# heliaxdev/ark-plonk

Hardware: AMD Instinct MI355X
Metric: proofs/sec at 2^20 constraints (BLS12-381, KZG10); MSM G1-adds/s (higher is better)
Workload: dtype u32 limbs (256/384-bit Montgomery integers)

## Files before the change

ark_plonk_amd/csrc/ecu.cuh:

```cuda
#pragma once
#include "fields.cuh"

template <class F>
struct AffineU {
    F x, y;
    ZK_HD bool is_null() const { return x.limbs_zero() && y.limbs_zero(); }
};

template <class F>
struct XYZZu {
    F x, y, zz, zzz;

    ZK_HD static XYZZu infinity() {
        XYZZu r;
        r.x = F::zero();
        r.y = F::zero();
        r.zz = F::zero();
        r.zzz = F::zero();
        return r;
    }
    ZK_HD bool is_inf() const { return zz.limbs_zero(); }

    ZK_HD static XYZZu from_affine(const AffineU<F>& p) {
        XYZZu r;
        r.x = p.x;
        r.y = p.y;
        r.zz = F::one();
        r.zzz = F::one();
        return r;
    }

    ZK_HD static XYZZu dbl_affine(const AffineU<F>& p) {
        F u = F::dbl(p.y);
        F v = F::sqr(u);
        F w = F::mul(u, v);
        F s = F::mul(p.x, v);
        F xx = F::sqr(p.x);
        F m = F::add3(xx, xx, xx);
        XYZZu r;
        r.x = F::sub8(F::sqr(m), F::dbl(s));
        r.y = F::dot2(m, F::sub16(s, r.x), w, F::neg16(p.y));
        r.zz = v;
        r.zzz = w;
        return r;
    }

    ZK_HD static XYZZu dbl(const XYZZu& p) {
        if (p.is_inf()) return p;
        F u = F::dbl(p.y);
        F v = F::sqr(u);
        F w = F::mul(u, v);
        F s = F::mul(p.x, v);
        F xx = F::sqr(p.x);
        F m = F::add3(xx, xx, xx);
        XYZZu r;
        r.x = F::sub8(F::sqr(m), F::dbl(s));
        r.y = F::dot2(m, F::sub16(s, r.x), w, F::neg16(p.y));
        r.zz = F::mul(v, p.zz);
        r.zzz = F::mul(w, p.zzz);
        return r;
    }

    ZK_HD static XYZZu madd(const XYZZu& p, const AffineU<F>& q) {
        if (p.is_inf()) return from_affine(q);
        F u2 = F::mul(q.x, p.zz);
        F s2 = F::mul(q.y, p.zzz);
        F pp_ = F::sub16(u2, p.x);
        F r_ = F::sub16(s2, p.y);
        F pp = F::sqr(pp_);
        F rr = F::sqr(r_);
        XYZZu o;
        o.zz = F::mul(p.zz, pp);
        if (o.zz.is_zero_mod_reduced()) {
            if (rr.is_zero_mod_reduced()) return dbl_affine(q);
            return infinity();
        }
        F ppp = F::mul(pp_, pp);
        F qq = F::mul(p.x, pp);
        o.x = F::sub_sum3(rr, ppp, qq, qq);
        o.y = F::dot2(r_, F::sub16(qq, o.x), F::neg16(p.y), ppp);
        o.zzz = F::mul(p.zzz, ppp);
        return o;
    }

    ZK_HD static XYZZu add(const XYZZu& p, const XYZZu& q) {
        if (p.is_inf()) return q;
        if (q.is_inf()) return p;
        F u1 = F::mul(p.x, q.zz);
        F u2 = F::mul(q.x, p.zz);
        F s1 = F::mul(p.y, q.zzz);
        F s2 = F::mul(q.y, p.zzz);
        F pp_ = F::sub8(u2, u1);
        F r_ = F::sub8(s2, s1);
        F pp = F::sqr(pp_);
        F rr = F::sqr(r_);
        XYZZu o;
        o.zz = F::mul(F::mul(p.zz, q.zz), pp);
        if (o.zz.is_zero_mod_reduced()) {
            if (rr.is_zero_mod_reduced()) return dbl(p);
            return infinity();
        }
        F ppp = F::mul(pp_, pp);
        F qq = F::mul(u1, pp);
        o.x = F::sub_sum3(rr, ppp, qq, qq);
        o.y = F::dot2(r_, F::sub16(qq, o.x), F::neg16(s1), ppp);
        o.zzz = F::mul(F::mul(p.zzz, q.zzz), ppp);
        return o;
    }

    ZK_HD bool to_affine(AffineU<F>& out) const {
        if (is_inf()) {
            out.x = F::zero();
            out.y = F::zero();
            return false;
        }
        F i3 = F::inverse(zzz);
        F zi = F::mul(zz, i3);
        F zi2 = F::sqr(zi);
        out.x = F::mul(x, zi2);
        out.y = F::mul(y, i3);
        return true;
    }
};
```

ark_plonk_amd/csrc/fields.cuh:

```cuda
#pragma once
#include "zk_common.h"

template <class P>
struct Fs {
    static constexpr int NL = P::NL;
    static constexpr int SAT = P::SAT_WORDS;
    static constexpr uint32_t M = (1u << 30) - 1u;
    static constexpr int32_t H = 1 << 29;
    uint32_t v[NL];

    ZK_HD static int32_t sx(uint32_t x) { return (int32_t)(x << 2) >> 2; }
    ZK_HD static int64_t column_bias() {
        int64_t h = H;
#if defined(__HIP_DEVICE_COMPILE__)
        asm volatile("" : "+s"(h));
#endif
        return h;
    }

    ZK_HD static Fs zero() {
        Fs r;
#pragma unroll
        for (int i = 0; i < NL; ++i) r.v[i] = 0;
        return r;
    }
    ZK_HD static Fs one() {
        Fs r;
#pragma unroll
        for (int i = 0; i < NL; ++i) r.v[i] = (uint32_t)P::ONE(i);
        return r;
    }
    ZK_HD bool limbs_zero() const {
        uint32_t o = 0;
#pragma unroll
        for (int i = 0; i < NL; ++i) o |= v[i];
        return o == 0;
    }

    ZK_HD static void normalize(Fs& t) {
        int32_t c = 0;
#pragma unroll
        for (int i = 0; i < NL - 1; ++i) {
            const int32_t x = (int32_t)t.v[i];
            const int32_t r = sx((uint32_t)x);
            t.v[i] = (uint32_t)(r + c);
            c = (x - r) >> 30;
        }
        t.v[NL - 1] += (uint32_t)c;
    }
    ZK_HD static void normalize_wide(Fs& t) {
        int32_t c = 0;
#pragma unroll
        for (int i = 0; i < NL - 1; ++i) {
            const int32_t x = (int32_t)t.v[i];
            t.v[i] = (uint32_t)(sx((uint32_t)x) + c);
            c = (x >> 30) + (int32_t)(((uint32_t)x >> 29) & 1u);
        }
        t.v[NL - 1] += (uint32_t)c;
    }
    ZK_HD static void normalize_strict(Fs& t) {
#pragma unroll
        for (int i = 0; i < NL - 1; ++i) {
            const int32_t x = (int32_t)t.v[i];
            const int32_t r = sx((uint32_t)x);
            t.v[i] = (uint32_t)r;
            t.v[i + 1] += (uint32_t)((x - r) >> 30);
        }
    }

    ZK_HD static Fs add(const Fs& a, const Fs& b) {
        Fs t;
#pragma unroll
        for (int i = 0; i < NL; ++i) t.v[i] = a.v[i] + b.v[i];
        normalize(t);
        return t;
    }
    ZK_HD static Fs dbl(const Fs& a) {
        Fs t;
#pragma unroll
        for (int i = 0; i < NL; ++i) t.v[i] = a.v[i] << 1;
        normalize(t);
        return t;
    }
    ZK_HD static Fs add3(const Fs& a, const Fs& b, const Fs& c) {
        Fs t;
#pragma unroll
        for (int i = 0; i < NL; ++i) t.v[i] = a.v[i] + b.v[i] + c.v[i];
        normalize_wide(t);
        return t;
    }
    ZK_HD static Fs sub(const Fs& a, const Fs& b) {
        Fs t;
#pragma unroll
        for (int i = 0; i < NL; ++i) t.v[i] = a.v[i] - b.v[i];
        normalize(t);
        return t;
    }
    ZK_HD static Fs sub_sum3(const Fs& a, const Fs& b, const Fs& c, const Fs& d) {
        Fs t;
#pragma unroll
        for (int i = 0; i < NL; ++i) t.v[i] = a.v[i] - b.v[i] - c.v[i] - d.v[i];
        normalize_wide(t);
        return t;
    }
    ZK_HD static Fs sub2(const Fs& a, const Fs& b) { return sub(a, b); }
    ZK_HD static Fs sub8(const Fs& a, const Fs& b) { return sub(a, b); }
    ZK_HD static Fs sub16(const Fs& a, const Fs& b) { return sub(a, b); }
    ZK_HD static Fs neg16(const Fs& a) {
        Fs t;
#pragma unroll
        for (int i = 0; i < NL; ++i) t.v[i] = 0u - a.v[i];
        return t;
    }
    ZK_HD static Fs neg_canonical(const Fs& a) { return neg16(a); }

    ZK_HD static Fs mul(const Fs& a, const Fs& b) {
        int32_t m[NL];
        Fs r;
        int64_t carry = 0;
        const int64_t hb = column_bias();
#pragma unroll
        for (int k = 0; k < NL; ++k) {
            int64_t a0 = 0, a1 = 0, am = 0;
#pragma unroll
            for (int i = 0; i <= k; ++i) {
                if (i & 1) a1 += (int64_t)(int32_t)a.v[i] * (int32_t)b.v[k - i];
                else a0 += (int64_t)(int32_t)a.v[i] * (int32_t)b.v[k - i];
            }
#pragma unroll
            for (int i = 0; i < k; ++i) am += (int64_t)m[i] * P::MOD(k - i);
            int64_t t = a0 + a1 + am + carry;
            m[k] = (int32_t)((uint32_t)t * (P::PINV << 2)) >> 2;
            t += (int64_t)m[k] * P::MOD(0);
            carry = t >> 30;
        }
#pragma unroll
        for (int k = NL; k < 2 * NL - 1; ++k) {
            int64_t a0 = hb, a1 = 0, am = 0;
#pragma unroll
            for (int i = k - NL + 1; i < NL; ++i) {
                if (i & 1) a1 += (int64_t)(int32_t)a.v[i] * (int32_t)b.v[k - i];
                else a0 += (int64_t)(int32_t)a.v[i] * (int32_t)b.v[k - i];
                am += (int64_t)m[i] * P::MOD(k - i);
            }
            const int64_t t = a0 + a1 + am + carry;
            r.v[k - NL] = ((uint32_t)t & M) - (uint32_t)H;
            carry = t >> 30;
        }
        r.v[NL - 1] = (uint32_t)carry;
        return r;
    }
    ZK_HD static Fs dot2(const Fs& a, const Fs& b, const Fs& c, const Fs& d) {
        int32_t m[NL];
        Fs r;
        int64_t carry = 0;
        const int64_t hb = column_bias();
#pragma unroll
        for (int k = 0; k < NL; ++k) {
            int64_t a0 = 0, a1 = 0, am = 0;
#pragma unroll
            for (int i = 0; i <= k; ++i) {
                a0 += (int64_t)(int32_t)a.v[i] * (int32_t)b.v[k - i];
                a1 += (int64_t)(int32_t)c.v[i] * (int32_t)d.v[k - i];
            }
#pragma unroll
            for (int i = 0; i < k; ++i) am += (int64_t)m[i] * P::MOD(k - i);
            int64_t t = a0 + a1 + am + carry;
            m[k] = (int32_t)((uint32_t)t * (P::PINV << 2)) >> 2;
            t += (int64_t)m[k] * P::MOD(0);
            carry = t >> 30;
        }
#pragma unroll
        for (int k = NL; k < 2 * NL - 1; ++k) {
            int64_t a0 = hb, a1 = 0, am = 0;
#pragma unroll
            for (int i = k - NL + 1; i < NL; ++i) {
                a0 += (int64_t)(int32_t)a.v[i] * (int32_t)b.v[k - i];
                a1 += (int64_t)(int32_t)c.v[i] * (int32_t)d.v[k - i];
                am += (int64_t)m[i] * P::MOD(k - i);
            }
            const int64_t t = a0 + a1 + am + carry;
            r.v[k - NL] = ((uint32_t)t & M) - (uint32_t)H;
            carry = t >> 30;
        }
        r.v[NL - 1] = (uint32_t)carry;
        return r;
    }
    ZK_HD static Fs sqr(const Fs& a) {
        int32_t m[NL], a2[NL];
        Fs r;
#pragma unroll
        for (int i = 0; i < NL; ++i) a2[i] = (int32_t)(a.v[i] << 1);
        int64_t carry = 0;
        const int64_t hb = column_bias();
#pragma unroll
        for (int k = 0; k < NL; ++k) {
            int64_t aa = 0, am = 0;
#pragma unroll
            for (int i = 0; 2 * i < k; ++i) aa += (int64_t)a2[i] * (int32_t)a.v[k - i];
            if ((k & 1) == 0) aa += (int64_t)(int32_t)a.v[k / 2] * (int32_t)a.v[k / 2];
#pragma unroll
            for (int i = 0; i < k; ++i) am += (int64_t)m[i] * P::MOD(k - i);
            int64_t t = aa + am + carry;
            m[k] = (int32_t)((uint32_t)t * (P::PINV << 2)) >> 2;
            t += (int64_t)m[k] * P::MOD(0);
            carry = t >> 30;
        }
#pragma unroll
        for (int k = NL; k < 2 * NL - 1; ++k) {
            int64_t aa = hb, am = 0;
#pragma unroll
            for (int i = k - NL + 1; 2 * i < k; ++i) aa += (int64_t)a2[i] * (int32_t)a.v[k - i];
            if ((k & 1) == 0) aa += (int64_t)(int32_t)a.v[k / 2] * (int32_t)a.v[k / 2];
#pragma unroll
            for (int i = k - NL + 1; i < NL; ++i) am += (int64_t)m[i] * P::MOD(k - i);
            const int64_t t = aa + am + carry;
            r.v[k - NL] = ((uint32_t)t & M) - (uint32_t)H;
            carry = t >> 30;
        }
        r.v[NL - 1] = (uint32_t)carry;
        return r;
    }

    ZK_HD bool is_zero_mod_reduced() const {
        if (v[0] != 0 && v[0] != (uint32_t)P::MOD(0) && v[0] != (uint32_t)P::NMOD(0)) return false;
        uint32_t dz = 0, dp = 0, dn = 0;
#pragma unroll
        for (int i = 0; i < NL; ++i) {
            dz |= v[i];
            dp |= v[i] ^ (uint32_t)P::MOD(i);
            dn |= v[i] ^ (uint32_t)P::NMOD(i);
        }
        return dz == 0 || dp == 0 || dn == 0;
    }
    ZK_HD bool is_zero_mod() const { return mul(*this, one()).is_zero_mod_reduced(); }

    ZK_HD static void floor_sweep(Fs& t) {
#pragma unroll
        for (int i = 0; i < NL - 1; ++i) {
            const int32_t x = (int32_t)t.v[i];
            t.v[i] = (uint32_t)x & M;
            t.v[i + 1] += (uint32_t)(x >> 30);
        }
    }
    ZK_HD static Fs canon_floor(const Fs& a) {
        Fs x = a;
        floor_sweep(x);
#pragma unroll
        for (int it = 0; it < 2; ++it) {
            Fs y;
#pragma unroll
            for (int i = 0; i < NL; ++i) y.v[i] = x.v[i] + (uint32_t)P::MOD(i);
            floor_sweep(y);
            const bool neg = (int32_t)x.v[NL - 1] < 0;
#pragma unroll
            for (int i = 0; i < NL; ++i) x.v[i] = neg ? y.v[i] : x.v[i];
        }
#pragma unroll
        for (int it = 0; it < 2; ++it) {
            Fs y;
#pragma unroll
            for (int i = 0; i < NL; ++i) y.v[i] = x.v[i] - (uint32_t)P::MOD(i);
            floor_sweep(y);
            const bool ge = (int32_t)y.v[NL - 1] >= 0;
#pragma unroll
            for (int i = 0; i < NL; ++i) x.v[i] = ge ? y.v[i] : x.v[i];
        }
        return x;
    }
    ZK_HD static Fs canonical_lt2p(const Fs& a) {
        Fs x = canon_floor(a);
        normalize_strict(x);
        return x;
    }

    ZK_HD static Fs from_sat(const uint32_t* w) {
        Fs t = split_words(w);
        Fs c;
#pragma unroll
        for (int i = 0; i < NL; ++i) c.v[i] = (uint32_t)P::C_IN(i);
        return mul(t, c);
    }
    ZK_HD void to_sat(uint32_t* w) const {
        Fs c;
#pragma unroll
        for (int i = 0; i < NL; ++i) c.v[i] = (uint32_t)P::C_OUT(i);
        canon_floor(mul(*this, c)).pack_words(w);
    }
    ZK_HD static Fs split_words(const uint32_t* w) {
        Fs t;
#pragma unroll
        for (int i = 0; i < NL; ++i) {
            const int bit = 30 * i;
            const int wi = bit >> 5, off = bit & 31;
            uint64_t lo = wi < SAT ? w[wi] : 0u;
            uint64_t hi = (wi + 1) < SAT ? w[wi + 1] : 0u;
            t.v[i] = (uint32_t)(((hi << 32) | lo) >> off) & M;
        }
        normalize_strict(t);
        return t;
    }
    ZK_HD void pack_words(uint32_t* w) const {
#pragma unroll
        for (int j = 0; j < SAT; ++j) {
            const int lo_bit = 32 * j;
            uint64_t acc = 0;
#pragma unroll
            for (int i = 0; i < NL; ++i) {
                const int lb = 30 * i;
                if (lb + 30 <= lo_bit || lb >= lo_bit + 32) continue;
                if (lb >= lo_bit) acc |= (uint64_t)v[i] << (lb - lo_bit);
                else acc |= (uint64_t)v[i] >> (lo_bit - lb);
            }
            w[j] = (uint32_t)acc;
        }
    }

    ZK_HD static Fs pow_words(const Fs& a, const uint32_t* e, int n) {
        Fs r = one();
        bool started = false;
        for (int i = n - 1; i >= 0; --i)
            for (int b = 31; b >= 0; --b) {
                if (started) r = sqr(r);
                if ((e[i] >> b) & 1u) {
                    r = mul(r, a);
                    started = true;
                }
            }
        return r;
    }
    ZK_HD static Fs inverse(const Fs& a) {
        uint32_t e[SAT];
#pragma unroll
        for (int i = 0; i < SAT; ++i) e[i] = P::MODW(i);
        uint64_t t = (uint64_t)e[0] - 2u;
        e[0] = (uint32_t)t;
        uint32_t borrow = (uint32_t)(t >> 32) & 1u;
        for (int i = 1; i < SAT && borrow; ++i) {
            t = (uint64_t)e[i] - borrow;
            e[i] = (uint32_t)t;
            borrow = (uint32_t)(t >> 32) & 1u;
        }
        return pow_words(a, e, SAT);
    }
};
```

ark_plonk_amd/csrc/msm_accumulate.hip:

```cpp
#include "msm_common.cuh"

namespace {

template <class F, bool PRE>
ZK_D void accumulate_chunk(const uint32_t t, const uint32_t* entries, const uint32_t* offsets, uint32_t nb, const void* bases, void* buckets,
                           void* part_pt, uint32_t L0, uint32_t n_lanes, uint64_t tab_stride, uint64_t tab_off) {
    const uint32_t E = offsets[nb];
    const uint32_t L = chunk_len(E, n_lanes, L0);
    const uint64_t e0 = (uint64_t)t * L;
    if (e0 >= E) return;
    const uint32_t e1 = (uint32_t)min((uint64_t)E, e0 + L);
    uint32_t lo = 0, hi = nb - 1;
    while (lo < hi) {
        uint32_t mid = (lo + hi + 1) >> 1;
        if (offsets[mid] <= (uint32_t)e0) lo = mid; else hi = mid - 1;
    }
    uint32_t b = lo;
    uint32_t bend = offsets[b + 1];
    const bool head_partial = offsets[b] < (uint32_t)e0;
    bool first_run = true;
    XYZZu<F> acc = XYZZu<F>::infinity();
    auto point_index = [&](uint32_t ref) -> uint64_t {
        return PRE ? (uint64_t)((ref >> 26) & 31u) * tab_stride + tab_off + (ref & 0x3ffffffu) : (uint64_t)(ref & 0x7fffffffu);
    };
    uint32_t ref_n = entries[(uint32_t)e0];
    AffineU<F> p_n = ld_affine<F>(bases, point_index(ref_n));
    for (uint32_t e = (uint32_t)e0; e < e1; ++e) {
        const uint32_t ref = ref_n;
        AffineU<F> p = p_n;
        if (e + 1 < e1) {
            ref_n = entries[e + 1];
            p_n = ld_affine<F>(bases, point_index(ref_n));
        }
        if (e == bend) {
            if (first_run && head_partial) st_xyzz<F>(part_pt, 2ull * t, acc);
            else st_xyzz<F>(buckets, b, acc);
            first_run = false;
            acc = XYZZu<F>::infinity();
            do {
                ++b;
                bend = offsets[b + 1];
            } while (bend <= e);
        }
        if (p.is_null()) continue;
        if (ref >> 31) p.y = F::neg_canonical(p.y);
        acc = XYZZu<F>::madd(acc, p);
    }
    const bool tail_complete = (e1 == bend);
    if (first_run) {
        if (head_partial || !tail_complete) st_xyzz<F>(part_pt, 2ull * t, acc);
        else st_xyzz<F>(buckets, b, acc);
    } else {
        if (tail_complete) st_xyzz<F>(buckets, b, acc);
        else st_xyzz<F>(part_pt, 2ull * t + 1, acc);
    }
}

template <class F, bool PRE>
__global__ void __launch_bounds__(128) msm_accumulate(const uint32_t* entries, const uint32_t* offsets, uint32_t nb, const void* bases,
                                                       void* buckets, void* part_pt, uint32_t L, uint32_t n_lanes, uint64_t tab_stride,
                                                       uint64_t tab_off) {
    const uint32_t t = blockIdx.x * blockDim.x + threadIdx.x;
    if (t >= n_lanes) return;
    accumulate_chunk<F, PRE>(t, entries, offsets, nb, bases, buckets, part_pt, L, n_lanes, tab_stride, tab_off);
}

template <class F>
__global__ void __launch_bounds__(128) msm_accumulate_batch(AJobs jobs, uint32_t nb, const void* bases, uint64_t tab_stride) {
    uint32_t k = 0;
    while (k + 1 < jobs.n && blockIdx.x >= jobs.j[k + 1].blk0) ++k;
    const AJob& J = jobs.j[k];
    const uint32_t t = (blockIdx.x - J.blk0) * blockDim.x + threadIdx.x;
    if (t >= J.n_lanes) return;
    accumulate_chunk<F, true>(t, J.entries, J.offsets, nb, bases, J.buckets, J.part_pt, J.L0, J.n_lanes, tab_stride, J.tab_off);
}

template <class Cv>
__global__ void bases_to_internal(const uint32_t* xy_sat, const uint8_t* inf, uint64_t n, void* out) {
    typedef typename Cv::FqU F;
    uint64_t i = (uint64_t)blockIdx.x * blockDim.x + threadIdx.x;
    if (i >= n) return;
    const uint32_t* w = xy_sat + i * 2 * F::SAT;
    uint32_t any_x = 0, y_not_zero = 0, y_not_one = 0;
    for (int k = 0; k < F::SAT; ++k) {
        any_x |= w[k];
        y_not_zero |= w[F::SAT + k];
        y_not_one |= w[F::SAT + k] ^ Cv::FqP::R(k);
    }
    uint4* q = reinterpret_cast<uint4*>(out) + i * (2 * Store<F>::U4);
    if ((any_x == 0 && (y_not_zero == 0 || y_not_one == 0)) || (inf && inf[i])) {
        st_fu<F>(q, F::zero());
        st_fu<F>(q + Store<F>::U4, F::zero());
        return;
    }
    st_fu<F>(q, F::canonical_lt2p(F::from_sat(w)));
    st_fu<F>(q + Store<F>::U4, F::canonical_lt2p(F::from_sat(w + F::SAT)));
}

template <class Cv>
__global__ void __launch_bounds__(128) g1_fixed_base(const uint32_t* scalars, uint64_t n, uint32_t* out_xy) {
    typedef typename Cv::FqU F;
    uint64_t i = (uint64_t)blockIdx.x * blockDim.x + threadIdx.x;
    if (i >= n) return;
    uint32_t gw[2 * F::SAT];
#pragma unroll
    for (int k = 0; k < F::SAT; ++k) {
        gw[k] = Cv::FqP::GX(k);
        gw[F::SAT + k] = Cv::FqP::GY(k);
    }
    AffineU<F> G;
    G.x = F::canonical_lt2p(F::from_sat(gw));
    G.y = F::canonical_lt2p(F::from_sat(gw + F::SAT));
    const uint32_t* s = scalars + 8 * i;
    XYZZu<F> acc = XYZZu<F>::infinity();
    for (int limb = 7; limb >= 0; --limb) {
        const uint32_t word = s[limb];
        for (int b = 31; b >= 0; --b) {
            acc = XYZZu<F>::dbl(acc);
            if ((word >> b) & 1u) acc = XYZZu<F>::madd(acc, G);
        }
    }
    AffineU<F> o;
    uint32_t* dst = out_xy + i * 2 * F::SAT;
    if (!acc.to_affine(o)) {
        for (int k = 0; k < 2 * F::SAT; ++k) dst[k] = 0;
        return;
    }
    o.x.to_sat(dst);
    o.y.to_sat(dst + F::SAT);
}

constexpr uint32_t CHAIN_RB = 32;
template <class F>
__global__ void __launch_bounds__(128) msm_precompute(void* table, const void* src, uint64_t n, uint32_t d0, uint32_t dstep, uint32_t rows, uint32_t out0,
                                                      void* scratch) {
    const uint64_t i = (uint64_t)blockIdx.x * blockDim.x + threadIdx.x;
    if (i >= n) return;
    constexpr int U4 = Store<F>::U4;
    uint4* base = reinterpret_cast<uint4*>(table);
    uint4* scr = reinterpret_cast<uint4*>(scratch);
    auto row = [&](uint32_t r) { return base + ((uint64_t)(out0 + r) * n + i) * (2 * U4); };
    auto sc = [&](uint32_t j, uint32_t which) { return scr + (((uint64_t)j * n + i) * 3 + which) * U4; };
    AffineU<F> p = ld_affine<F>(src, i);
    if (p.is_null()) {
        for (uint32_t r = 0; r < rows; ++r) {
            st_fu<F>(row(r), F::zero());
            st_fu<F>(row(r) + U4, F::zero());
        }
        return;
    }
    XYZZu<F> acc = XYZZu<F>::from_affine(p);
    for (uint32_t r0 = 0; r0 < rows; r0 += CHAIN_RB) {
        const uint32_t m = rows - r0 < CHAIN_RB ? rows - r0 : CHAIN_RB;
        F prefix = F::one();
        for (uint32_t j = 0; j < m; ++j) {
            const uint32_t nd = r0 + j == 0 ? d0 : dstep;
            for (uint32_t k = 0; k < nd; ++k) acc = XYZZu<F>::dbl(acc);
            st_fu<F>(row(r0 + j), acc.x);
            st_fu<F>(row(r0 + j) + U4, acc.y);
            st_fu<F>(sc(j, 0), acc.zz);
            st_fu<F>(sc(j, 1), acc.zzz);
            prefix = F::mul(prefix, acc.zzz);
            st_fu<F>(sc(j, 2), prefix);
        }
        F inv = F::inverse(prefix);
        for (uint32_t j = m; j-- > 0;) {
            const F zzz = ld_fu<F>(sc(j, 1));
            const F i3 = j ? F::mul(inv, ld_fu<F>(sc(j - 1, 2))) : inv;
            inv = F::mul(inv, zzz);
            const F zi = F::mul(ld_fu<F>(sc(j, 0)), i3);
            const F zi2 = F::sqr(zi);
            const F x = F::canonical_lt2p(F::mul(ld_fu<F>(row(r0 + j)), zi2));
            const F y = F::canonical_lt2p(F::mul(ld_fu<F>(row(r0 + j) + U4), i3));
            st_fu<F>(row(r0 + j), x);
            st_fu<F>(row(r0 + j) + U4, y);
        }
    }
}

template <class Cv>
int msm_precompute_run(zk_ctx* c, zk_srs* s, uint32_t window_bits, uint32_t w0, uint32_t wstep) {
    typedef typename Cv::FqU F;
    if (window_bits == 0) window_bits = (s->n >= (1u << 22) && wstep == 1) ? 20 : s->n >= (1u << 19) ? PRE_C + 1 : PRE_C;
    if (window_bits < PRE_C || window_bits > PRE_C_MAX) return ZK_ERR_BAD_ARG;
    MsmGeom g = make_geom<typename Cv::FrP>(1u << 20, (int)window_bits, PRE_C_MAX);
    if (wstep == 0 || w0 >= wstep || w0 >= g.W) return ZK_ERR_BAD_ARG;
    const uint32_t rows = (g.W - w0 + wstep - 1) / wstep;
    const bool whole = wstep == 1;
    const size_t pb = s->point_bytes;
    void* tab = nullptr;
    void* scratch = nullptr;
    if (hipMalloc(&tab, (size_t)rows * s->n * pb) != hipSuccess) {
        (void)hipGetLastError();
        return ZK_ERR_OOM;
    }
    const uint32_t out0 = w0 == 0 ? 1u : 0u, chain_rows = rows - out0;
    const uint32_t rb = chain_rows < CHAIN_RB ? chain_rows : CHAIN_RB;
    if (hipMalloc(&scratch, (size_t)(rb ? rb : 1) * s->n * 3 * (pb / 2)) != hipSuccess) {
        (void)hipGetLastError();
        (void)hipFree(tab);
        return ZK_ERR_OOM;
    }
    hipError_t e = hipSuccess;
    if (w0 == 0) e = hipMemcpyAsync(tab, s->d_xy, s->n * pb, hipMemcpyDeviceToDevice, c->stream);
    if (e == hipSuccess && chain_rows) {
        const int T = 128;
        unsigned blocks = (unsigned)((s->n + T - 1) / T);
        hipLaunchKernelGGL(msm_precompute<F>, dim3(blocks), dim3(T), 0, c->stream, tab, (const void*)s->d_xy, (uint64_t)s->n,
                           w0 == 0 ? g.c * wstep : g.c * w0, g.c * wstep, chain_rows, out0, scratch);
        e = hipGetLastError();
    }
    if (e == hipSuccess) e = hipStreamSynchronize(c->stream);
    (void)hipFree(scratch);
    if (e != hipSuccess) {
        (void)hipFree(tab);
        zk_note_hip_error(e, "msm_precompute", __FILE__, __LINE__);
        return ZK_ERR_HIP;
    }
    if (whole) {
        (void)hipFree(s->d_xy);
        s->d_xy = tab;
    } else {
        s->d_pre = tab;
    }
    s->pre_c = g.c;
    s->pre_W = g.W;
    s->pre_rows = rows;
    s->pre_w0 = w0;
    s->pre_wstep = wstep;
    return ZK_OK;
}


template <class Cv>
int pw_queue_accumulate(zk_ctx* c, const MsmGeom& g, MsmBufs& mb, const void* d_bases, uint32_t n_lanes, hipStream_t st) {
    typedef typename Cv::FqU F;
    ProfScope ps(c, "msm_accumulate", st);
    const int T = 128;
    unsigned blocks = (n_lanes + T - 1) / T;
    hipLaunchKernelGGL((msm_accumulate<F, false>), dim3(blocks), dim3(T), 0, st, (const uint32_t*)mb.entries.p, (const uint32_t*)mb.offsets.p, g.nb, d_bases,
                       mb.buckets.p, mb.part_pt.p, CHUNK_L, n_lanes, (uint64_t)0, (uint64_t)0);
    ZK_HIP_TRY(hipGetLastError());
    return ZK_OK;
}

template <class Cv>
int pre_queue_accumulate(zk_ctx* c, const PrePlan* pls, MsmBufs* const* mbs, const size_t* lens, const size_t* tab_offs, uint32_t n_jobs, zk_srs* s,
                         hipStream_t st) {
    typedef typename Cv::FqU F;
    if (n_jobs == 0) return ZK_OK;
    if (n_jobs > (uint32_t)MAX_JOBS) return ZK_ERR_UNSUPPORTED;
    ProfScope ps(c, "msm_accumulate", st);
    const uint32_t T = 128;
    AJobs aj;
    memset(&aj, 0, sizeof aj);
    aj.n = n_jobs;
    uint64_t blocks = 0, points = 0;
    for (uint32_t k = 0; k < n_jobs; ++k) {
        MsmBufs& mb = *mbs[k];
        AJob& J = aj.j[k];
        J.entries = (const uint32_t*)mb.entries.p;
        J.offsets = (const uint32_t*)mb.offsets.p;
        J.buckets = mb.buckets.p;
        J.part_pt = mb.part_pt.p;
        J.tab_off = tab_offs ? tab_offs[k] : 0;
        J.L0 = pls[k].chunk_l;
        J.n_lanes = pls[k].n_lanes;
        mb.acc_chunk_l = pls[k].chunk_l;
        mb.acc_n_lanes = pls[k].n_lanes;
        J.blk0 = (uint32_t)blocks;
        blocks += (pls[k].n_lanes + T - 1) / T;
        points += lens[k];
    }
    if (blocks >= (1ull << 31)) return ZK_ERR_UNSUPPORTED;
    if (c->profiling) {
        c->prof["msm_accumulate_jobs"].launches += n_jobs;
        c->prof["msm_accumulate_points"].launches += points;
    }
    hipLaunchKernelGGL(msm_accumulate_batch<F>, dim3((unsigned)blocks), dim3(T), 0, st, aj, pls[0].g1.nb, s->table(), (uint64_t)s->n);
    ZK_HIP_TRY(hipGetLastError());
    return ZK_OK;
}

}

int ZK_SYM(pw_queue_accumulate)(zk_ctx* c, const MsmGeom& g, MsmBufs& mb, const void* d_bases, uint32_t n_lanes, hipStream_t st) {
    return pw_queue_accumulate<CurveSel>(c, g, mb, d_bases, n_lanes, st);
}
int ZK_SYM(pre_queue_accumulate)(zk_ctx* c, const PrePlan* pls, MsmBufs* const* mbs, const size_t* lens, const size_t* tab_offs, uint32_t n_jobs, zk_srs* s,
                                 hipStream_t st) {
    return pre_queue_accumulate<CurveSel>(c, pls, mbs, lens, tab_offs, n_jobs, s, st);
}

int ZK_SYM(msm_fixed_base_dev)(zk_ctx* c, const void* d_scalars, size_t n, void* d_out_xy) {
    if (n == 0) return ZK_OK;
    const int T = 128;
    unsigned blocks = (unsigned)((n + T - 1) / T);
    hipLaunchKernelGGL(g1_fixed_base<CurveSel>, dim3(blocks), dim3(T), 0, c->stream, (const uint32_t*)d_scalars, (uint64_t)n,
                       (uint32_t*)d_out_xy);
    ZK_HIP_TRY(hipGetLastError());
    return ZK_OK;
}

int ZK_SYM(msm_convert_bases_dev)(zk_ctx* c, const void* d_xy_sat, const uint8_t* d_inf, size_t n, void* d_out_internal) {
    if (n == 0) return ZK_OK;
    const int T = 256;
    unsigned blocks = (unsigned)((n + T - 1) / T);
    hipLaunchKernelGGL(bases_to_internal<CurveSel>, dim3(blocks), dim3(T), 0, c->stream, (const uint32_t*)d_xy_sat, d_inf, (uint64_t)n,
                       d_out_internal);
    ZK_HIP_TRY(hipGetLastError());
    return ZK_OK;
}

int ZK_SYM(msm_precompute_dev)(zk_ctx* c, zk_srs* s, uint32_t window_bits, uint32_t w0, uint32_t wstep) {
    return msm_precompute_run<CurveSel>(c, s, window_bits, w0, wstep);
}

size_t ZK_SYM(msm_point_bytes)() { return (size_t)2 * Store<CurveSel::FqU>::WORDS * 4; }
size_t ZK_SYM(msm_partial_dev_bytes)() { return (size_t)4 * Store<CurveSel::FqU>::WORDS * 4; }
```

Measured before the change: 11.87.

## Split mixed addition and overlap next base load with its second half

Restructures the bucket accumulation loop so the mixed point addition is split into a first half (two multiplications) and a finish stage. The load of the next affine base is issued between the two halves, replacing the previous software-prefetch register copy. Infinity is now tracked with an explicit flag instead of testing limbs, and the rare doubling case reloads the current point. The added predication hints and flag logic aim to cut register pressure and hide memory latency, at the cost of more divergent control flow.

New measurement: 12.05, median of 6. 1.01x the previous value.

```diff
diff --git a/ark_plonk_amd/csrc/ecu.cuh b/ark_plonk_amd/csrc/ecu.cuh
--- a/ark_plonk_amd/csrc/ecu.cuh
+++ b/ark_plonk_amd/csrc/ecu.cuh
@@ -1,5 +1,12 @@
 #pragma once
 #include "fields.cuh"
+
+ZK_HD bool zk_apart(uint32_t flag) {
+#if defined(__HIP_DEVICE_COMPILE__)
+    asm volatile("" : "+v"(flag));
+#endif
+    return flag != 0;
+}
 
 template <class F>
 struct AffineU {
@@ -83,6 +90,36 @@
         return o;
     }
 
+    enum : int { MADD_SUM = 0, MADD_SAME = 1, MADD_OPPOSITE = 2 };
+    struct MaddHalf {
+        F u2, s2;
+    };
+    ZK_HD static MaddHalf madd_begin(const XYZZu& p, const AffineU<F>& q) {
+        MaddHalf h;
+        h.u2 = F::mul(q.x, p.zz);
+        h.s2 = F::mul(q.y, p.zzz);
+        return h;
+    }
+    ZK_HD static int madd_finish(XYZZu& p, const MaddHalf& h) {
+        F pp_ = F::sub16(h.u2, p.x);
+        F r_ = F::sub16(h.s2, p.y);
+        F pp = F::sqr(pp_);
+        F rr = F::sqr(r_);
+        p.zz = F::mul(p.zz, pp);
+        int how = MADD_SUM;
+        if (p.zz.limb0_of_zero_mod()) {
+            if (p.zz.is_zero_mod_reduced()) how = rr.is_zero_mod_reduced() ? MADD_SAME : MADD_OPPOSITE;
+        }
+        if (zk_apart(how == MADD_SUM)) {
+            F ppp = F::mul(pp_, pp);
+            F qq = F::mul(p.x, pp);
+            p.x = F::sub_sum3(rr, ppp, qq, qq);
+            p.y = F::dot2(r_, F::sub16(qq, p.x), F::neg16(p.y), ppp);
+            p.zzz = F::mul(p.zzz, ppp);
+        }
+        return how;
+    }
+
     ZK_HD static XYZZu add(const XYZZu& p, const XYZZu& q) {
         if (p.is_inf()) return q;
         if (q.is_inf()) return p;
diff --git a/ark_plonk_amd/csrc/fields.cuh b/ark_plonk_amd/csrc/fields.cuh
--- a/ark_plonk_amd/csrc/fields.cuh
+++ b/ark_plonk_amd/csrc/fields.cuh
@@ -222,6 +222,7 @@
         return r;
     }
 
+    ZK_HD bool limb0_of_zero_mod() const { return v[0] == 0 || v[0] == (uint32_t)P::MOD(0) || v[0] == (uint32_t)P::NMOD(0); }
     ZK_HD bool is_zero_mod_reduced() const {
         if (v[0] != 0 && v[0] != (uint32_t)P::MOD(0) && v[0] != (uint32_t)P::NMOD(0)) return false;
         uint32_t dz = 0, dp = 0, dn = 0;
diff --git a/ark_plonk_amd/csrc/msm_accumulate.hip b/ark_plonk_amd/csrc/msm_accumulate.hip
--- a/ark_plonk_amd/csrc/msm_accumulate.hip
+++ b/ark_plonk_amd/csrc/msm_accumulate.hip
@@ -20,39 +20,63 @@
     const bool head_partial = offsets[b] < (uint32_t)e0;
     bool first_run = true;
     XYZZu<F> acc = XYZZu<F>::infinity();
+    bool inf = true;
+    auto store_run = [&](void* arr, uint64_t slot) {
+        if (inf) acc = XYZZu<F>::infinity();
+        st_xyzz<F>(arr, slot, acc);
+    };
     auto point_index = [&](uint32_t ref) -> uint64_t {
         return PRE ? (uint64_t)((ref >> 26) & 31u) * tab_stride + tab_off + (ref & 0x3ffffffu) : (uint64_t)(ref & 0x7fffffffu);
     };
-    uint32_t ref_n = entries[(uint32_t)e0];
-    AffineU<F> p_n = ld_affine<F>(bases, point_index(ref_n));
+    uint32_t ref = entries[(uint32_t)e0];
+    AffineU<F> p = ld_affine<F>(bases, point_index(ref));
     for (uint32_t e = (uint32_t)e0; e < e1; ++e) {
-        const uint32_t ref = ref_n;
-        AffineU<F> p = p_n;
-        if (e + 1 < e1) {
-            ref_n = entries[e + 1];
-            p_n = ld_affine<F>(bases, point_index(ref_n));
-        }
+        const uint32_t ref_n = entries[e + 1 < e1 ? e + 1 : e];
         if (e == bend) {
-            if (first_run && head_partial) st_xyzz<F>(part_pt, 2ull * t, acc);
-            else st_xyzz<F>(buckets, b, acc);
+            if (first_run && head_partial) store_run(part_pt, 2ull * t);
+            else store_run(buckets, b);
             first_run = false;
-            acc = XYZZu<F>::infinity();
+            inf = true;
             do {
                 ++b;
                 bend = offsets[b + 1];
             } while (bend <= e);
         }
-        if (p.is_null()) continue;
-        if (ref >> 31) p.y = F::neg_canonical(p.y);
-        acc = XYZZu<F>::madd(acc, p);
+        const bool point = !p.is_null();
+        const bool add = zk_apart(point && !inf);
+        if (zk_apart(point && inf)) {
+            acc.x = p.x;
+            acc.y = (ref >> 31) ? F::neg_canonical(p.y) : p.y;
+            acc.zz = F::one();
+            acc.zzz = F::one();
+            inf = false;
+        }
+        typename XYZZu<F>::MaddHalf h;
+        if (add) {
+            if (ref >> 31) p.y = F::neg_canonical(p.y);
+            h = XYZZu<F>::madd_begin(acc, p);
+        }
+        p = ld_affine<F>(bases, point_index(ref_n));
+        int how = XYZZu<F>::MADD_SUM;
+        if (zk_apart(add)) how = XYZZu<F>::madd_finish(acc, h);
+        if (zk_apart(how != XYZZu<F>::MADD_SUM)) {
+            if (how == XYZZu<F>::MADD_SAME) {
+                AffineU<F> q = ld_affine<F>(bases, point_index(ref));
+                if (ref >> 31) q.y = F::neg_canonical(q.y);
+                acc = XYZZu<F>::dbl_affine(q);
+            } else {
+                inf = true;
+            }
+        }
+        ref = ref_n;
     }
     const bool tail_complete = (e1 == bend);
     if (first_run) {
-        if (head_partial || !tail_complete) st_xyzz<F>(part_pt, 2ull * t, acc);
-        else st_xyzz<F>(buckets, b, acc);
+        if (head_partial || !tail_complete) store_run(part_pt, 2ull * t);
+        else store_run(buckets, b);
     } else {
-        if (tail_complete) st_xyzz<F>(buckets, b, acc);
-        else st_xyzz<F>(part_pt, 2ull * t + 1, acc);
+        if (tail_complete) store_run(buckets, b);
+        else store_run(part_pt, 2ull * t + 1);
     }
 }
 
```
